# lucanest/Phyloformer

Hardware: AMD Instinct MI355X
Metric: alignments/sec, 60-leaf/500-site LG+GC-like MSAs, Phyloformer forward (pf.ckpt) (higher is better)
Workload: dtype f16x3-split MFMA (two fp16 limbs per operand, 3 passes), fp32 accumulate/residual

## Files before the change

### phyloformer_amd/csrc/pf_device.hip.h

```cpp
#pragma once
#include <hip/hip_runtime.h>
#include <stdint.h>

#include "pf_layout.h"

namespace pfk {

typedef float f32x4 __attribute__((ext_vector_type(4)));
typedef float f32x16 __attribute__((ext_vector_type(16)));
#if PF_F16
typedef _Float16 h16_t;
#define PF_MFMA(a, b, c) __builtin_amdgcn_mfma_f32_32x32x16_f16((a), (b), (c), 0, 0, 0)
#define PF_DOT2C "v_dot2c_f32_f16"
#define PF_CVT_PK "v_cvt_pk_f16_f32"
#define PF_NEG1_LO 0x0000bc00u
#define PF_NEG1_HI 0xbc000000u
#else
typedef __bf16 h16_t;
#define PF_MFMA(a, b, c) __builtin_amdgcn_mfma_f32_32x32x16_bf16((a), (b), (c), 0, 0, 0)
#define PF_DOT2C "v_dot2c_f32_bf16"
#define PF_CVT_PK "v_cvt_pk_bf16_f32"
#define PF_NEG1_LO 0x0000bf80u
#define PF_NEG1_HI 0xbf800000u
#endif
// ... 296 lines not shown
    int nt_aln;
    int slots_aln;
    size_t trash_tok;
    int store_x_last;
    unsigned long long* prof;
    int ablate;
    float* sitemap;
    const float* w;
};

enum { MODE_FIRST = 0, MODE_MID = 1, MODE_LAST = 2, MODE_MID0 = 3, MODE_LAST_FOLD = 4 };

struct TilePos { int b, kt, r0, l0; };
template <bool FLAT>
__device__ __forceinline__ TilePos tile_pos(const MainArgs& a, int task, int ntiles) {
    TilePos q;
    q.b = task / a.nt_aln;
    q.kt = task - q.b * a.nt_aln;
    if (FLAT) { const int tok0 = q.kt * 32; q.r0 = tok0 / a.Lloc; q.l0 = tok0 - q.r0 * a.Lloc; }
    else { q.r0 = q.kt / ntiles; q.l0 = (q.kt - q.r0 * ntiles) * 32; }
    return q;
}
template <bool FLAT>
__device__ __forceinline__ TilePos tile_next(const MainArgs& a, TilePos q) {
    if (++q.kt == a.nt_aln) { q.b++; q.kt = 0; q.r0 = 0; q.l0 = 0; return q; }
    q.l0 += 32;
    if (q.l0 >= a.Lloc) { q.l0 = FLAT ? q.l0 - a.Lloc : 0; q.r0++; }
    return q;
}
struct LanePos { size_t tok0; int toff, l, nvalid, wrap; bool valid, in_r1; };
template <bool FLAT>
__device__ __forceinline__ LanePos lane_pos(const MainArgs& a, const TilePos& q, int t) {
    LanePos o;
    o.tok0 = ((size_t)q.b * a.P + q.r0) * a.Lloc + q.l0;
    const int left = FLAT ? a.P * a.Lloc - q.kt * 32 : a.Lloc - q.l0;
    o.nvalid = min(32, left);
    o.wrap = (FLAT && q.r0 + 1 < a.P) ? min(32, a.Lloc - q.l0) : 32;
    o.valid = t < o.nvalid;
    o.toff = min(t, o.nvalid - 1);
    o.in_r1 = o.toff >= o.wrap;
    o.l = q.l0 + o.toff - (o.in_r1 ? a.Lloc : 0);
    return o;
}
__device__ __forceinline__ void part_range(int flat, int pr, int nparts, int P, int L, int slots_aln, long* first, int* count) {
    if (!flat) { *first = (long)pr * nparts; *count = nparts; return; }
    const int b = pr / P, p = pr - b * P;
    const int k0 = (int)(((long)p * L) >> 5), k1 = (int)((((long)p + 1) * L - 1) >> 5);
    *first = (long)b * slots_aln + k0 + p;
    *count = k1 - k0 + 1;
}

template <int LO, int HI>
__device__ __forceinline__ void image_to_lds(const frag_t* src, unsigned char* smem) {
    static_assert(LO % 64 == 0 && HI % 64 == 0, "the image is copied in whole waves");
    const int wv = threadIdx.x >> 6, ln = threadIdx.x & 63;
#pragma unroll
    for (int k = 0; k < (HI - LO + MAIN_THREADS - 1) / MAIN_THREADS; ++k) {
        const int f0 = LO + k * MAIN_THREADS + wv * 64;
        if (f0 < HI) __builtin_amdgcn_global_load_lds(src + f0 + ln, smem + (size_t)f0 * 16, 16, 0, 0);
    }
}

template <int MODE, bool FLAT, bool SITEMAP = false, bool WEIGHTED = false>
__global__ void __launch_bounds__(MAIN_THREADS, MAIN_WAVES / 4) k_main(MainArgs a) {
    constexpr bool LAST = MODE == MODE_LAST || MODE == MODE_LAST_FOLD;
    constexpr bool FOLD = MODE == MODE_LAST_FOLD;
    static_assert(!SITEMAP || LAST, "the site map is the head's: last block only");
    static_assert(!WEIGHTED || (!SITEMAP && MODE != MODE_FIRST), "weighted launches: blocks' own modes, no site map");
    extern __shared__ __attribute__((aligned(16))) unsigned char smem[];
    lds_frag_t lw = (lds_frag_t)smem;
    lds_f32_t lc = (lds_f32_t)(smem + FRAG_END * 16);

    {
        const float cv = a.consts[min((int)threadIdx.x, CONST_LEN - 1)];
        if (FOLD) {
            image_to_lds<FRAG_W1, FRAG_W2>(a.wimg, smem);
            image_to_lds<FRAG_WO, FRAG_U + U_FRAGS>(a.wimg, smem);
        } else {
            image_to_lds<(MODE == MODE_FIRST) ? FRAG_WV : 0, LAST ? FRAG_WV : FRAG_END>(a.wimg, smem);
        }
        static_assert(CONST_LEN <= MAIN_THREADS, "one constant per thread");
        if (threadIdx.x < CONST_LEN) reinterpret_cast<float*>(smem + FRAG_END * 16)[threadIdx.x] = cv;
        asm volatile("s_waitcnt vmcnt(0)" ::: "memory");
    }
    __syncthreads();

    const int lane = threadIdx.x & 63;
    const int wave = __builtin_amdgcn_readfirstlane(threadIdx.x >> 6);
    const int t = lane & 31;
    const int h = lane >> 5;
    const int ntiles = (a.Lloc + 31) >> 5;
    const int ntasks = a.B * a.nt_aln;
    if (wave >= MAIN_WAVES / 2) __builtin_amdgcn_s_setprio(1);
    unsigned long long tacc[6] = {0, 0, 0, 0, 0, 0}, tprev = 0;
#define PF_TICK(k) do { if (a.prof) { const unsigned long long tn_ = __builtin_amdgcn_s_memtime(); tacc[k] += tn_ - tprev; tprev = tn_; } } while (0)
    if (a.prof) tprev = __builtin_amdgcn_s_memtime();
    lds_frag_t w1p = lw + FRAG_W1 + lane;
    lds_frag_t w2p = lw + FRAG_W2 + lane;
    lds_frag_t wop = lw + FRAG_WO + lane;
    lds_frag_t qkp = lw + FRAG_QK + h * 8 + (t & 7);
    lds_f32_t lch = lc + 4 * h;
    PF_OPAQUE(wop); PF_OPAQUE(qkp); PF_OPAQUE(lch);
    lds_frag_t wvp = wop + (FRAG_WV - FRAG_WO);
    lds_f32_t luh = (lds_f32_t)(smem + FRAG_U * 16) + 16 * h;

    {
        const int nwaves = gridDim.x * MAIN_WAVES;
#ifndef PF_RUN_MAX
#define PF_RUN_MAX 8
#endif
        const int run = max(1, min(PF_RUN_MAX, ntasks / (nwaves * 8)));
        int run0 = (blockIdx.x * MAIN_WAVES + wave) * run;
        const int task0 = run0, task1 = ntasks;
        TilePos cur = tile_pos<FLAT>(a, min(task0, ntasks - 1), ntiles);
        int frag_row = -1;
        frag_t mfr[4];
        f32x4 rqv = {0.f, 0.f, 0.f, 0.f};
        f32x4 px[8], pctx[8], pqr, pqc;
        int pri = 0, prj = 0;
        auto prefetch = [&](const TilePos& np) {
            const LanePos nl = lane_pos<FLAT>(a, np, t);
            const int ll = nl.l, pb = np.b;
            const size_t tk = nl.tok0 + nl.toff;
            if (MODE == MODE_MID0) {
                const uint8_t* ib = a.idx + (size_t)pb * a.N * a.Lloc + ll;
                const int pp = np.r0 + (nl.in_r1 ? 1 : 0);
                pri = residue(ib[(size_t)a.pair_i[pp] * a.Lloc]);
                prj = residue(ib[(size_t)a.pair_j[pp] * a.Lloc]);
            } else {
                const f32x4* xp = reinterpret_cast<const f32x4*>(a.x + tk * 64 + 4 * h);
#pragma unroll
                for (int g = 0; g < 8; ++g) px[g] = xp[2 * g];
            }
            pqr = *reinterpret_cast<const f32x4*>(a.qrow + tk * 4);
            pqc = *reinterpret_cast<const f32x4*>(a.qcol + tk * 4);
            if (MODE != MODE_FIRST) {
                int hq = h;
                asm volatile("" : "+v"(hq));
                const f32x4* cp = reinterpret_cast<const f32x4*>(a.ctx + ((size_t)pb * a.Lloc + ll) * 64 + 4 * hq);
#pragma unroll
                for (int g = 0; g < 8; ++g) pctx[g] = cp[2 * g];
            }
        };
        if (MODE != MODE_FIRST && task0 < task1) prefetch(cur);

        for (int task = task0; task < task1;) {
            const int b = cur.b;
            const int row = b * a.P + cur.r0;
            int ntask = task + 1;
            TilePos nxt = tile_next<FLAT>(a, cur);
            if (ntask == run0 + run) {
                run0 += nwaves * run;
                ntask = run0;
                if (ntask < task1) nxt = tile_pos<FLAT>(a, ntask, ntiles);
            }
            const LanePos lp = lane_pos<FLAT>(a, cur, t);
            const bool straddle = lp.wrap < 32;
            int ai = 0, aj = 0;
            if (MODE == MODE_FIRST) { const int pp = cur.r0 + (lp.in_r1 ? 1 : 0); ai = a.pair_i[pp]; aj = a.pair_j[pp]; }
            auto load_mfr = [&](int r) {
                const frag_t* mf = a.mfrag + (size_t)r * 128 + t;
#pragma unroll
                for (int q = 0; q < 4; ++q) mfr[q] = mf[q * 32];
                typedef const f32x4 __attribute__((address_space(4)))* const_f32x4_t;
                rqv = *(const_f32x4_t)(unsigned long long)(a.rq + (size_t)__builtin_amdgcn_readfirstlane(r) * 4);
                frag_row = r;
            };
            if (MODE != MODE_FIRST && row != frag_row) load_mfr(row);
            const bool valid = lp.valid;
            const int lc_ = lp.l;
            const size_t tok = lp.tok0 + lp.toff;
            float x[32];
            float zh[4] = {0.f, 0.f, 0.f, 0.f};
            float wt = 1.f;
            if (WEIGHTED && LAST) wt = a.w[(size_t)b * a.Lloc + lc_];

            if (MODE == MODE_FIRST) {
                const int ri = residue(a.idx[((size_t)b * a.N + ai) * a.Lloc + lc_]);
                const int rj = residue(a.idx[((size_t)b * a.N + aj) * a.Lloc + lc_]);
                const f32x4* ti = reinterpret_cast<const f32x4*>(a.table + ri * 64 + 4 * h);
                const f32x4* tj = reinterpret_cast<const f32x4*>(a.table + rj * 64 + 4 * h);
#pragma unroll
                for (int g = 0; g < 8; ++g) {
                    f32x4 u = ti[2 * g], w = tj[2 * g];
#pragma unroll
                    for (int i = 0; i < 4; ++i) x[4 * g + i] = u[i] + w[i];
                }
            } else {
                if (MODE == MODE_MID0) {
                    const f32x4* ti = reinterpret_cast<const f32x4*>(a.table + pri * 64 + 4 * h);
                    const f32x4* tj = reinterpret_cast<const f32x4*>(a.table + prj * 64 + 4 * h);
#pragma unroll
                    for (int g = 0; g < 8; ++g) {
                        const f32x4 u = ti[2 * g], w = tj[2 * g];
#pragma unroll
                        for (int i = 0; i < 4; ++i) x[4 * g + i] = u[i] + w[i];
                    }
                } else {
#pragma unroll
                    for (int g = 0; g < 8; ++g)
#pragma unroll
                        for (int i = 0; i < 4; ++i) x[4 * g + i] = px[g][i];
                }
                PF_TICK(0);
                if (!(a.ablate & 8)) {
                    f32x16 ya[2];
#pragma unroll
                    for (int j = 0; j < 32; ++j) ya[j >> 4][j & 15] = x[j];
                    {
                        const f32x4 qr = pqr;
                        auto mix = [&](const bool mine) {
                            float v[8];
#pragma unroll
                            for (int i = 0; i < 4; ++i) v[i] = mine ? qr[i] * rqv[i] : 0.f;
                            v[4] = v[5] = mine ? 1.f : 0.f;
                            v[6] = v[7] = 0.f;
                            frag_t qb_hi, qb_lo;
                            split8(v, qb_hi, qb_lo);
#pragma unroll
                            for (int To = 0; To < 2; ++To) mfma3(ya[To], mfr[To * 2], mfr[To * 2 + 1], qb_hi, qb_lo, To == 1);
                        };
                        mix(h == 0 && !lp.in_r1);
                        if (straddle) {
                            load_mfr(row + 1);
                            mix(h == 0 && lp.in_r1);
                        }
                    }
                    {
                        const f32x4 qc = pqc * COLAPPLY_B_SCALE;
                        float o[32];
#pragma unroll
                        for (int g = 0; g < 8; ++g) {
                            const f32x4 u = pctx[g];
#pragma unroll
                            for (int i = 0; i < 4; ++i) o[4 * g + i] = u[i] * qc[g >> 1];
                        }
#pragma unroll
                        for (int s = 0; s < 4; ++s) {
                            frag_t ob_hi, ob_lo;
                            split8(&o[8 * s], ob_hi, ob_lo);
#pragma unroll
                            for (int To = 0; To < 2; ++To) {
                                lds_frag_t f = wop + ((To * 4 + s) * 2) * 64;
                                const frag_t a_hi = f[0], a_lo = f[64];
                                mfma3(ya[To], a_hi, a_lo, ob_hi, ob_lo, To == 1);
                            }
                        }
                    }
#pragma unroll
                    for (int j = 0; j < 32; ++j) x[j] = ya[j >> 4][j & 15];
                }

                PF_TICK(1);
                if (FOLD) {
#pragma unroll
                    for (int g = 0; g < 8; ++g) {
                        const f32x4 w4 = *(lds_f32x4_t)(lch + CONST_HW + 8 * g);
#pragma unroll
                        for (int i = 0; i < 4; ++i) zh[i] = fmaf(w4[i], x[4 * g + i], zh[i]);
                    }
                }
                if (FOLD && !(a.ablate & 16)) {
                    frag_t xb_hi[4], xb_lo[4];
                    {
                        float xn[32];
                        ln_pair(x, xn);
#pragma unroll
                        for (int s = 0; s < 4; ++s) split8(&xn[8 * s], xb_hi[s], xb_lo[s]);
                    }
                    if (ntask < task1) prefetch(nxt);
                    PF_TICK(2);
#pragma unroll 1
                    for (int T = 0; T < 8; ++T) {
                        f32x16 ha;
                        lds_frag_t f1 = w1p + T * 512;
                        lds_f32_t bp = lch + CONST_B1 + 32 * T;
                        lds_f32_t up = luh + 32 * T;
                        PF_OPAQUE(f1); PF_OPAQUE(bp); PF_OPAQUE(up);
// ... 43 lines not shown
                            frag_t nh, nl;
                            if (s < 3) { nh = f1[(s + 1) * 128]; nl = f1[(s + 1) * 128 + 64]; }
                            else { nh = f2[0]; nl = f2[64]; }
                            mfma3(ha, fh, fl, xb_hi[s], xb_lo[s]);
                            fh = nh; fl = nl;
                        }
                        frag_t g_hi[2], g_lo[2];
                        gelu_split8(ha, 0, g_hi[0], g_lo[0]);
                        gelu_split8(ha, 8, g_hi[1], g_lo[1]);
#pragma unroll
                        for (int st = 0; st < 4; ++st) {
                            const int u = st >> 1, To = st & 1;
                            frag_t nh = fh, nl = fl;
                            if (st < 3) {
                                const int nu = (st + 1) >> 1, nTo = (st + 1) & 1;
                                nh = f2[(nTo * 32 + nu * 2) * 64];
                                nl = f2[(nTo * 32 + nu * 2) * 64 + 64];
                            }
                            mfma3(oa[To], fh, fl, g_hi[u], g_lo[u], To == 1);
                            fh = nh; fl = nl;
                        }
                    }
                    PF_TICK(3);
#pragma unroll
                    for (int j = 0; j < 32; ++j) x[j] = oa[j >> 4][j & 15];
                }
            }

            if (!LAST && !(a.ablate & 4)) {
                frag_t wl[8];
#pragma unroll
                for (int i = WVLO_LDS; i < 8; ++i) wl[i] = a.wv_lo[i * 64 + lane];
                if (WEIGHTED) wt = a.w[(size_t)b * a.Lloc + lc_];
                __builtin_amdgcn_sched_barrier(0);
                {
                    const size_t stok = valid ? tok : a.trash_tok + t;
                    f32x4* xo = reinterpret_cast<f32x4*>(a.x + stok * 64 + 4 * h);
#pragma unroll
                    for (int g = 0; g < 8; ++g) {
                        f32x4 u = {x[4 * g], x[4 * g + 1], x[4 * g + 2], x[4 * g + 3]};
                        xo[2 * g] = u;
                    }
                }
                if (a.ablate & 32) { cur = nxt; task = ntask; continue; }
                f32x16 va[3];
                {
                    float xn[32];
                    ln_pair(x, xn);
                    frag_t xb_hi[4], xb_lo[4];
#pragma unroll
                    for (int s = 0; s < 4; ++s) split8(&xn[8 * s], xb_hi[s], xb_lo[s]);
#pragma unroll
                    for (int s = 0; s < 4; ++s) {
                        const frag_t q_hi = qkp[(s * 2) * 16], q_lo = qkp[(s * 2 + 1) * 16];
                        if (s == 0) mfma3_zero(va[2], q_hi, q_lo, xb_hi[s], xb_lo[s]);
                        else mfma3(va[2], q_hi, q_lo, xb_hi[s], xb_lo[s]);
                    }
#pragma unroll
                    for (int s = 0; s < 4; ++s)
#pragma unroll
                        for (int T = 0; T < 2; ++T) {
                            const frag_t f_hi = wvp[(T * 4 + s) * 64];
                            const frag_t f_lo = T * 4 + s < WVLO_LDS ? wvp[(FRAG_WVLO - FRAG_WV) + (T * 4 + s) * 64] : wl[T * 4 + s];
                            if (s == 0) mfma3_zero(va[T], f_hi, f_lo, xb_hi[s], xb_lo[s], T == 1);
                            else mfma3(va[T], f_hi, f_lo, xb_hi[s], xb_lo[s], T == 1);
                        }
                }
#pragma unroll
                for (int r = 0; r < 4; ++r) va[2][r] += lc[CONST_BQK + 4 * h + r];
                float qk[4], ot[4];
#pragma unroll
                for (int i = 0; i < 4; ++i) qk[i] = elu1_fast(va[2][i]);
#pragma unroll
                for (int i = 0; i < 4; ++i) ot[i] = pair_other(qk[i], h);
                float qn[4], kn[4];
#pragma unroll
                for (int i = 0; i < 4; ++i) {
                    qn[i] = h ? ot[i] : qk[i];
                    kn[i] = h ? qk[i] : ot[i];
                }
                {
                    const size_t stok = valid ? tok : a.trash_tok + t;
                    f32x4 qs = {qn[0], qn[1], qn[2], qn[3]};
                    *reinterpret_cast<f32x4*>(a.qrow + stok * 4) = qs;
                }
                const long slot0 = (long)b * a.slots_aln + cur.kt + (FLAT ? cur.r0 : 0);
                for (int part = 0; part < (straddle ? 2 : 1); ++part) {
                    float* sp = a.spart + (size_t)(slot0 + part) * SROW;
                    const float vm = (valid && lp.in_r1 == (part == 1)) ? (WEIGHTED ? wt : 1.f) : 0.f;
                    float km[4];
#pragma unroll
                    for (int i = 0; i < 4; ++i) km[i] = kn[i] * vm;
                    {
                        float qk8[8];
#pragma unroll
                        for (int i = 0; i < 4; ++i) { qk8[i] = vm * qn[i]; qk8[4 + i] = km[i]; }
                        const float sqk = treduce8(qk8, t);
                        if (lane < 8) sp[64 + lane] = sqk;
                    }
                    {
                        float kv[32];
#pragma unroll
                        for (int j = 0; j < 32; ++j) kv[j] = km[j >> 3] * va[j >> 4][j & 15];
                        sp[kmap(t, h)] = treduce32(kv, t);
                    }
                }
            } else if (LAST) {
                float z = 0.f;
                if (FOLD) {
                    z = pair_sum((zh[0] + zh[1]) + (zh[2] + zh[3])) + lc[CONST_C0];
                } else {
#pragma unroll
                    for (int g = 0; g < 8; ++g) {
                        const f32x4 w4 = *(lds_f32x4_t)(lch + CONST_HW + 8 * g);
#pragma unroll
                        for (int i = 0; i < 4; ++i) z = fmaf(w4[i], x[4 * g + i], z);
                    }
                    z = pair_sum(z) + lc[CONST_HB];
                }
                const float spz = softplus20(z);
                const long slot0 = (long)b * a.slots_aln + cur.kt + (FLAT ? cur.r0 : 0);
                for (int part = 0; part < (straddle ? 2 : 1); ++part) {
// ... 614 lines not shown
                    n[u] = gg < a.G ? (min(a.npairs, (gg + 1) * per) - gg * per + a.sub - 1) / a.sub : 0;
                    nmax = max(nmax, n[u]);
                    pg[u] = pp + (size_t)gg * a.S * gs;
                    t[u] = 0.f;
                }
                for (int s = 0; s < nmax; s += 4) {
                    float v[GU][4];
#pragma unroll
                    for (int u = 0; u < GU; ++u)
#pragma unroll
                        for (int q = 0; q < 4; ++q)
                            v[u][q] = s + q < n[u] ? pg[u][(size_t)(s + q) * gs] : 0.f;
#pragma unroll
                    for (int u = 0; u < GU; ++u) t[u] = (((t[u] + v[u][0]) + v[u][1]) + v[u][2]) + v[u][3];
                }
#pragma unroll
                for (int u = 0; u < GU; ++u)
                    if (g + u < a.G) acc += t[u];
            }
        } else {
            const float* pp = a.part + ((size_t)b * a.G * a.Lloc + l) * CPART + i;
            int g = 0;
            for (; g + 4 <= a.G; g += 4) {
                const float v0 = pp[(size_t)g * gs], v1 = pp[(size_t)(g + 1) * gs], v2 = pp[(size_t)(g + 2) * gs],
                            v3 = pp[(size_t)(g + 3) * gs];
                acc = (((acc + v0) + v1) + v2) + v3;
            }
            for (; g < a.G; ++g) acc += pp[(size_t)g * gs];
        }
        zs[i] = acc;
    }
    __syncthreads();
    if (i < 256) {
        const float* z = zs + (hd >> 4) * 64 + 16 * quarter;
        float acc = 0.f;
#pragma unroll
        for (int k = 0; k < 16; ++k) acc = fmaf(w[k], z[k], acc);
        dp[quarter][hd] = acc;
    }
    __syncthreads();
    if (i < 64) {
        const int hh = hd >> 4;
        const float acc = ((dp[0][hd] + dp[1][hd]) + dp[2][hd]) + dp[3][hd];
        const float sq = zs[256 + hh], sk = zs[260 + hh];
        a.ctx[(size_t)site * 64 + hd] = (acc + a.bv[hd] * sk) / sk * (a.P / sq);
    }
}

__global__ void k_accumulate(float* dst, const float* src, size_t n) {
    const size_t i = (size_t)blockIdx.x * blockDim.x + threadIdx.x;
    if (i < n) dst[i] += src[i];
}

__global__ void k_selftest(float* out) {
    const int lane = threadIdx.x;
    out[lane] = pair_sum((float)lane);
    out[64 + lane] = pair_other((float)lane, lane >> 5);
    out[128 + lane] = row16_sum((float)lane);
    out[192 + lane] = half32_sum((float)lane);
    frag_t A1, A2, Bf;
    const int m = lane & 31, kg = lane >> 5;
#pragma unroll
    for (int i = 0; i < 8; ++i) {
        const int k = 8 * kg + i;
        A1[i] = (h16_t)(float)(m + 32 * (k % 8));
        A2[i] = (h16_t)(float)k;
        Bf[i] = (h16_t)((k == (m & 15)) ? 1.f : 0.f);
    }
    f32x16 acc1, acc2;
#pragma unroll
    for (int r = 0; r < 16; ++r) { acc1[r] = 0.f; acc2[r] = 0.f; }
    acc1 = PF_MFMA(A1, Bf, acc1);
    acc2 = PF_MFMA(A2, Bf, acc2);
#pragma unroll
    for (int r = 0; r < 16; ++r) {
        out[256 + lane * 16 + r] = acc1[r];
        out[1280 + lane * 16 + r] = acc2[r];
    }
}

#endif

}
```

### phyloformer_amd/csrc/pf_host_prep.h

```cpp
#pragma once
#include <algorithm>
#include <cmath>
#include <cstdint>
#include <cstring>
#include <vector>

#include "pf_layout.h"

namespace pfhost {
using namespace pfk;

inline uint16_t f2bf(float f) {
    uint32_t u;
    std::memcpy(&u, &f, 4);
    if ((u & 0x7fffffffu) > 0x7f800000u) return uint16_t((u >> 16) | 0x40);
    u += 0x7fffu + ((u >> 16) & 1u);
    return uint16_t(u >> 16);
}
inline float bf2f(uint16_t b) {
    uint32_t u = uint32_t(b) << 16;
    float f;
    std::memcpy(&f, &u, 4);
    return f;
}
// ... 5 lines not shown
    if (u >= 0x7f800000u) return uint16_t(sign | 0x7c00u | (u > 0x7f800000u ? 0x200u : 0u));
    if (u >= 0x477ff000u) return uint16_t(sign | 0x7c00u);
    if (u < 0x33000001u) return sign;
    const int e = int(u >> 23) - 127;
    uint32_t m = (u & 0x7fffffu) | 0x800000u;
    int shift = (e < -14) ? (13 + (-14 - e)) : 13;
    const uint32_t half = 1u << (shift - 1), rest = m & ((1u << shift) - 1);
    uint32_t r = m >> shift;
    if (rest > half || (rest == half && (r & 1u))) ++r;
    const uint32_t out = (e < -14) ? r : (uint32_t(e + 14) << 10) + r;
    return uint16_t(sign | out);
}
inline float h2f(uint16_t hbits) {
    const uint32_t sign = uint32_t(hbits & 0x8000u) << 16;
    const int e = (hbits >> 10) & 0x1f;
    const uint32_t m = hbits & 0x3ffu;
    float mag;
    if (e == 0) mag = std::ldexp((float)m, -24);
    else if (e == 31) mag = m ? NAN : INFINITY;
    else mag = std::ldexp((float)(m | 0x400u), e - 25);
    uint32_t u;
    std::memcpy(&u, &mag, 4);
    u |= sign;
    std::memcpy(&mag, &u, 4);
    return mag;
}
#if PF_F16
inline uint16_t f2x(float f) { return f2h(f); }
inline float x2f(uint16_t b) { return h2f(b); }
#else
inline uint16_t f2x(float f) { return f2bf(f); }
inline float x2f(uint16_t b) { return bf2f(b); }
#endif
inline int kmap_h(int j, int h) { return 8 * (j >> 2) + 4 * h + (j & 3); }

inline void pack_frags(const float* W, int M, int K, int Mpad, uint16_t* out, float scale = 1.f) {
    const int nT = Mpad / 32, nS = K / 16;
    for (int T = 0; T < nT; ++T)
        for (int s = 0; s < nS; ++s)
            for (int lane = 0; lane < 64; ++lane)
                for (int i = 0; i < 8; ++i) {
                    const int m = 32 * T + (lane & 31), k = kmap_h(8 * s + i, lane >> 5);
                    const float w = (m < M) ? W[(size_t)m * K + k] * scale : 0.f;
                    const uint16_t hi = f2x(w);
                    const uint16_t lo = f2x(w - x2f(hi));
                    const size_t base = ((size_t)(T * nS + s) * 2) * 64;
                    out[(base + lane) * 8 + i] = hi;
                    out[(base + 64 + lane) * 8 + i] = lo;
                }
}

inline void pack_qk_frags(const float* wq, const float* wk, uint16_t* qk) {
    for (int s = 0; s < 4; ++s)
        for (int kg = 0; kg < 2; ++kg)
            for (int m = 0; m < 8; ++m)
                for (int i = 0; i < 8; ++i) {
                    const int k = kmap_h(8 * s + i, kg);
                    const float w = (m < 4) ? wq[(size_t)m * E + k] : wk[(size_t)(m - 4) * E + k];
                    const uint16_t hi = f2x(w), lo = f2x(w - x2f(hi));
                    qk[(((size_t)s * 2 + 0) * 16 + kg * 8 + m) * 8 + i] = hi;
                    qk[(((size_t)s * 2 + 1) * 16 + kg * 8 + m) * 8 + i] = lo;
                }
}

inline void pack_row_stats(const float* wv, const float* wq, const float* wk, uint16_t* img_tail ,
                    uint16_t* wv_lo) {
    std::vector<uint16_t> full((size_t)2 * 4 * 2 * 64 * 8);
    pack_frags(wv, E, E, E, full.data());
    for (int T = 0; T < 2; ++T)
        for (int s = 0; s < 4; ++s)
            for (int lane = 0; lane < 64; ++lane)
                for (int i = 0; i < 8; ++i) {
                    const size_t src = (((size_t)(T * 4 + s) * 2) * 64 + lane) * 8 + i;
                    const size_t dst = ((size_t)(T * 4 + s) * 64 + lane) * 8 + i;
                    img_tail[dst] = full[src];
                    wv_lo[dst] = full[src + 64 * 8];
                }
    pack_qk_frags(wq, wk, img_tail + (size_t)(FRAG_QK - FRAG_WV) * 8);
}

inline void fold_head(const float* w2 , const float* b2, const float* hw, float hb, double w2_scale,
                      float* u_img , float* c0) {
    for (int T = 0; T < FF / 32; ++T)
        for (int h = 0; h < 2; ++h)
            for (int r = 0; r < 16; ++r) {
                const int k = 32 * T + kmap_h(r, h);
                double acc = 0.0;
                for (int c = 0; c < E; ++c) acc += (double)hw[c] * (double)w2[(size_t)c * FF + k];
                u_img[(T * 2 + h) * 16 + r] = (float)(acc * w2_scale);
            }
    double acc = (double)hb;
    for (int c = 0; c < E; ++c) acc += (double)hw[c] * (double)b2[c];
    *c0 = (float)acc;
}

struct AttnHost {
    const float *g, *b, *wq, *bq, *wk, *bk, *wv, *bv, *wo, *bo;
};
struct FfnHost {
    const float *g, *b, *w1, *b1, *w2, *b2;
};

struct BlobView {
    const float *emb_w, *emb_b;
    std::vector<AttnHost> row, col;
    std::vector<FfnHost> ffn;
    const float *head_w, *head_b;
    size_t len;
};
inline BlobView read_blob(const float* blob, int n_blocks, int E, int NH) {
    BlobView v{};
    const size_t e = (size_t)E, h = (size_t)NH;
    auto take = [&](size_t n) { const float* p = blob ? blob + v.len : nullptr; v.len += n; return p; };
    auto attn = [&] {
        AttnHost a;
// ... 112 lines not shown
```

### phyloformer_amd/csrc/pf_layout.h

```cpp
#pragma once

#ifndef PF_F16
#define PF_F16 1
#endif

namespace pfk {

constexpr int E = 64;
constexpr int NH = 4;
constexpr int HD = 16;
constexpr int FF = 256;
constexpr int NA = 22;
constexpr int SROW = 72;
constexpr int MROW = 4 * 64;
constexpr float LN_EPS = 1e-5f;

constexpr int FRAG_W1 = 0;
constexpr int FRAG_W2 = FRAG_W1 + 8 * 4 * 2 * 64;
constexpr int FRAG_WO = FRAG_W2 + 2 * 16 * 2 * 64;
constexpr int FRAG_WV = FRAG_WO + 2 * 4 * 2 * 64;
constexpr int FRAG_QK = FRAG_WV + 2 * 4 * 64;
#ifndef PF_WVLO_LDS
#define PF_WVLO_LDS 4
#endif
constexpr int WVLO_LDS = PF_WVLO_LDS;
constexpr int FRAG_WVLO = FRAG_QK + 4 * 2 * 16;
constexpr int FRAG_END = FRAG_WVLO + WVLO_LDS * 64;
constexpr int FRAG_U = FRAG_WV;
constexpr int U_FRAGS = FF * 4 / 16;
static_assert(FRAG_U + U_FRAGS <= FRAG_END, "the folded head fits the last block's tail");
constexpr int WVLO_FRAGS = 2 * 4 * 64;
constexpr int CONST_B1 = 0, CONST_B2 = 256, CONST_BQK = 320, CONST_HW = 328, CONST_HB = 392,
              CONST_C0 = 393, CONST_BOC = 400;
constexpr int CONST_LEN = 464;
constexpr int MAIN_LDS_BYTES = FRAG_END * 16 + CONST_LEN * 4;
constexpr int MFRAG_PER_PAIR = 2 * 2 * 32;

constexpr int MAIN_THREADS = 512;
constexpr int MAIN_WAVES = MAIN_THREADS / 64;

constexpr int PAIRTAB_ROWS = 22 * 22, PAIRTAB_W = 72;

}
```

### phyloformer_amd/csrc/pf_lib.hip

```cpp
#include <hip/hip_runtime.h>
#include <dlfcn.h>

#include <algorithm>
#include <cmath>
#include <cstdarg>
#include <cstdio>
#include <cstdlib>
#include <cstring>
#include <functional>
#include <map>
#include <mutex>
#include <string>
#include <type_traits>
#include <vector>

#include "../../include/phyloformer_amd.h"
#include "pf_device.hip.h"
#include "pf_mha.hip.h"
#include "pf_precise.hip.h"
#include "pf_generic.hip.h"
#include "pf_boot.hip.h"
#include "pf_sites.hip.h"
#include "pf_sitemap.hip.h"
#include "pf_sites_host.h"
// ... 603 lines not shown
        EmbedArgs e{r.d_idx, h->pair_i, h->pair_j, h->pair_table, h->table, x0, r.w.qrow, r.w.srow,
                    r.B, r.N, r.P, r.Lloc, h->bad_idx_dev, r.d_w};
        const int ntasks = r.B * r.P, wpb = EMBED_THREADS / 64;
        const int grid = std::max(1, std::min(h->prop.multiProcessorCount, (ntasks + wpb - 1) / wpb));
        ProfScope ps(h, K_EMBED);
        if (r.d_w) hipLaunchKernelGGL(k_embed<true>, dim3(grid), dim3(EMBED_THREADS), EMBED_LDS_BYTES, h->cur, e);
        else hipLaunchKernelGGL(k_embed<false>, dim3(grid), dim3(EMBED_THREADS), EMBED_LDS_BYTES, h->cur, e);
        HIPCHK(h, hipGetLastError());
    }
    if (h->debug_keep) return save_tap(h, "x0", r.w.x, (size_t)r.B * r.P * r.Lloc * 64);
    return PF_OK;
}

int tiles_of(int Lloc) { return (Lloc + 31) / 32; }

int launch_rowsum(pf_handle* h, const ShardRun& r, RowStats* rs) {
    if (rs->p == r.w.srow) return PF_OK;
    const int n = r.B * r.P * SROW;
    if (!r.Lloc) { *rs = RowStats{r.w.srow, 1, 0}; return zero_fill(h, r.w.srow, n); }
    ProfScope ps(h, K_ROWFIN);
    hipLaunchKernelGGL(k_rowsum, dim3((n + 255) / 256), dim3(256), 0, h->cur, rs->p, r.w.srow, r.B * r.P, rs->nparts,
                       rs->flat, r.P, r.Lloc, r.tp.slots_aln);
    HIPCHK(h, hipGetLastError());
    *rs = RowStats{r.w.srow, 1, 0};
    return PF_OK;
}

int launch_outsum(pf_handle* h, const ShardRun& r) {
    const int n = r.B * r.P;
    if (!r.Lloc) return zero_fill(h, r.d_out, n);
    ProfScope ps(h, K_ROWFIN);
    const TilePlan& tp = r.tp;
    hipLaunchKernelGGL(k_outsum, dim3((n + 255) / 256), dim3(256), 0, h->cur, r.w.outpart, r.d_out, n,
                       tiles_of(r.Lloc), 1.0f / (float)r.L_total, tp.flat, r.P, r.Lloc, tp.slots_aln, r.d_wst);
    HIPCHK(h, hipGetLastError());
    return PF_OK;
}

RowStats main_stats(const ShardRun& r) { return RowStats{r.w.spart, tiles_of(r.Lloc), r.tp.flat}; }

RowStats first_stats(pf_handle* h, const ShardRun& r) {
    return h->embed_mfma ? main_stats(r) : RowStats{r.w.srow, 1, 0};
}

int phase_block(pf_handle* h, const ShardRun& r, int k, RowStats rs) {
    if (!r.Lloc) return PF_OK;
    const BlockDev& d = h->blk[k];
    const Workspace& w = r.w;
    const int B = r.B, P = r.P, Lloc = r.Lloc;
    int rc;
    if (h->debug_keep) {
        if ((rc = launch_rowsum(h, r, &rs))) return rc;
        if ((rc = save_tap(h, "srow" + std::to_string(k), rs.p, (size_t)B * P * SROW))) return rc;
    }
    {
        RowFinArgs a{rs.p, w.mrow, reinterpret_cast<frag_t*>(w.mfrag),
                     d.row_woT, d.row_bv, d.row_bo, d.col_bo,
                     B * P, rs.nparts, (float)r.L_total, rs.flat, P, Lloc, r.tp.slots_aln, 1};
        const int groups = (B * P + 3) / 4;
        a.iters = std::max(1, std::min(16, groups / (4 * 8 * std::max(1, h->prop.multiProcessorCount))));
        a.rq = w.rq;
        a.b_scale = 1.f;
        for (long lim = 16384; lim < (long)r.L_total && a.b_scale > 1.f / 256.f; lim *= 2) a.b_scale *= 0.5f;
        a.a_scale = 1.f / a.b_scale;
        a.wst = r.d_wst;
        ProfScope ps(h, K_ROWFIN);
        hipLaunchKernelGGL(k_rowfin, dim3((groups + a.iters - 1) / a.iters), dim3(256), 0, h->cur, a);
        HIPCHK(h, hipGetLastError());
    }
    {
        ColStatsArgs a{w.x, w.qrow, w.mrow, w.qcol, w.part, d.col_wqk, d.col_bqk, d.row_bo, B, P, Lloc, w.G, (Lloc + 31) / 32,
                       w.sub, w.S, w.fine, h->table, r.d_idx, h->pair_i, h->pair_j, r.N};
        ProfScope ps(h, K_COLSTATS);
        const unsigned nblk = (unsigned)(B * a.nchunks * w.nparts());
        if (k == 0 && x0_on_the_fly(h))
            hipLaunchKernelGGL((k_colstats<true, 0, 16>), dim3(nblk), dim3(256), 0, h->cur, a);
        else if (h->colstats_ring)
            hipLaunchKernelGGL((k_colstats<false, PF_CS_RING, PF_CS_MT>), dim3(nblk), dim3(256), 0, h->cur, a);
        else
            hipLaunchKernelGGL((k_colstats<false, 0, 16>), dim3(nblk), dim3(256), 0, h->cur, a);
        HIPCHK(h, hipGetLastError());
    }
    {
        ColFinArgs a{w.part, w.ctx, d.col_wvT, d.col_bv, B, Lloc, w.G, (float)P, P, w.sub, w.S, w.fine};
        ProfScope ps(h, K_COLFIN);
        hipLaunchKernelGGL(k_colfin, dim3(B * Lloc), dim3(COLFIN_THREADS), 0, h->cur, a);
        HIPCHK(h, hipGetLastError());
    }
    if (h->debug_keep) {
        if ((rc = save_tap(h, "ctx" + std::to_string(k), w.ctx, (size_t)B * Lloc * 64))) return rc;
        if ((rc = save_tap(h, "mrow" + std::to_string(k), w.mrow, (size_t)B * P * MROW))) return rc;
    }
    MainArgs m = main_args(h, r);
    m.wimg = reinterpret_cast<const frag_t*>(d.wimg);
    m.consts = d.consts;
    if (k + 1 < h->n_blocks) {
        m.wv_lo = reinterpret_cast<const frag_t*>(h->blk[k + 1].wv_lo);
        const bool first = k == 0 && x0_on_the_fly(h);
        if (r.d_w) rc = first ? launch_main<MODE_MID0, false, true>(h, m, K_MAIN) : launch_main<MODE_MID, false, true>(h, m, K_MAIN);
        else rc = first ? launch_main<MODE_MID0>(h, m, K_MAIN) : launch_main<MODE_MID>(h, m, K_MAIN);
        if (rc) return rc;
    } else {
        m.wv_lo = nullptr;
        if (h->phase_prof_last) m.prof = h->phase_prof;
        m.sitemap = r.d_smap;
        if (!h->head_fold) {
// ... 2183 lines not shown
    if (!h) return PF_EINVAL;
    if (domain) *domain = h->prop.pciDomainID;
    if (bus) *bus = h->prop.pciBusID;
    if (device) *device = h->prop.pciDeviceID;
    return PF_OK;
}

int pf_forward_shards_emulated(pf_handle_t* h, const uint8_t* idx, int32_t B, int32_t N, int32_t L,
                               int32_t nshards, float* out) {
    if (!h) return PF_EINVAL;
    int rc = check_dims(h, B, N, L, L);
    if (rc) return rc;
    if (nshards < 1 || nshards > 64 || !idx || !out) return fail(h, PF_EINVAL, "bad shard count or null buffer");
    HIPCHK(h, hipSetDevice(h->device));
    if (const F64Path* f = f64_path_of(h, N, L)) return forward_shards_emulated_f64(h, *f, idx, B, N, L, nshards, out);
    if ((rc = ensure_pairs(h, N))) return rc;
    const int P = N * (N - 1) / 2;
    ShardStage stage(h);
    if ((rc = stage.upload(idx, B, N, L, nshards))) return rc;
    std::vector<ShardRun> runs;
    for (const ShardStage::Shard& s : stage.shards) {
        ShardRun r{{}, s.d_idx, nullptr, B, N, P, s.Lloc, L, tile_plan(h, P, s.Lloc), h->stream, {}};
        size_t off[WS_BUFS];
        char* ws = (char*)stage.alloc(workspace_bytes(h, B, P, r.Lloc, &r.w, off));
        r.d_out = (float*)stage.alloc((size_t)B * P * sizeof(float));
        if (!ws || !r.d_out) return fail(h, PF_ENOMEM, "shard workspace allocation failed");
        carve_workspace(ws, off, &r.w);
        runs.push_back(r);
    }
    float* total = (float*)stage.alloc((size_t)B * P * SROW * sizeof(float));
    if (!total) return fail(h, PF_ENOMEM, "shard sum buffer");
    auto reduce = [&](bool site_sums) -> int {
        const size_t count = (size_t)B * P * (site_sums ? 1 : SROW);
        for (ShardRun& r : runs)
            if (!site_sums && (rc = launch_rowsum(h, r, &r.rs))) return rc;
        hipMemsetAsync(total, 0, count * sizeof(float), h->stream);
        for (ShardRun& r : runs) {
            hipLaunchKernelGGL(k_accumulate, dim3((unsigned)((count + 255) / 256)), dim3(256), 0, h->stream,
                               total, site_sums ? r.d_out : r.w.srow, count);
            r.rs = RowStats{total, 1, 0};
        }
        return PF_OK;
    };
    rc = schedule(h, runs.data(), runs.size(), reduce);
    if (!rc && (hipMemcpyAsync(out, total, (size_t)B * P * sizeof(float), hipMemcpyDeviceToHost, h->stream) != hipSuccess ||
                hipStreamSynchronize(h->stream) != hipSuccess))
        rc = fail(h, PF_EHIP, "result copy failed");
    return rc;
}

int pf_selftest(pf_handle_t* h, float* out) {
    if (!h || !out) return PF_EINVAL;
    float* d = nullptr;
    HIPCHK(h, hipMalloc((void**)&d, 2304 * sizeof(float)));
    hipLaunchKernelGGL(k_selftest, dim3(1), dim3(64), 0, h->stream, d);
    HIPCHK(h, hipGetLastError());
    HIPCHK(h, hipMemcpyAsync(out, d, 2304 * sizeof(float), hipMemcpyDeviceToHost, h->stream));
    HIPCHK(h, hipStreamSynchronize(h->stream));
    hipFree(d);
    return PF_OK;
}

struct pf_mha {
    pf_handle* h = nullptr;
    float* wfrag = nullptr;
    float* bias = nullptr;
    std::vector<DeviceBuffer*> buffers;
    Buffer<char> ws{buffers};
    Buffer<float> d_x{buffers}, d_y{buffers};
};

int pf_mha_create(pf_handle_t* h, const pf_mha_weights_t* w, pf_mha_t** out) {
    if (!h || !w || !out) return PF_EINVAL;
    if (w->n_heads != MHA_H || w->embed_dim != E)
        return fail(h, PF_EINVAL, "softmax attention kernels are specialised for embed_dim 64 / 4 heads, got %d / %d",
                    w->embed_dim, w->n_heads);
    const float* ws[4] = {w->wq, w->wk, w->wv, w->wo};
    const float* bs[4] = {w->bq, w->bk, w->bv, w->bo};
    std::vector<uint16_t> img((size_t)MHA_WTOTAL * 8);
    std::vector<float> bias(4 * E);
    for (int i = 0; i < 4; ++i) {
        if (!ws[i] || !bs[i]) return fail(h, PF_EINVAL, "pf_mha_create: NULL weight pointer");
        std::copy(bs[i], bs[i] + E, bias.begin() + i * E);
    }
    pack_frags(w->wq, E, E, E, img.data());
    pack_frags(w->wk, E, E, E, img.data() + (size_t)MHA_OFF_WK * 8);
    pack_frags(w->wv, E, E, E, img.data() + (size_t)MHA_OFF_WV * 8);
    pack_frags(w->wo, E, E, E, img.data() + (size_t)MHA_OFF_WO * 8);
    HIPCHK(h, hipSetDevice(h->device));
    pf_mha* m = new pf_mha();
    m->h = h;
    void* p = nullptr;
    if (hipMalloc(&p, img.size() * 2) != hipSuccess) { delete m; return fail(h, PF_ENOMEM, "pf_mha_create: hipMalloc failed"); }
    m->wfrag = (float*)p;
    if (hipMalloc(&p, bias.size() * 4) != hipSuccess) { hipFree(m->wfrag); delete m; return fail(h, PF_ENOMEM, "pf_mha_create: hipMalloc failed"); }
    m->bias = (float*)p;
    if (hipMemcpy(m->wfrag, img.data(), img.size() * 2, hipMemcpyHostToDevice) != hipSuccess ||
        hipMemcpy(m->bias, bias.data(), bias.size() * 4, hipMemcpyHostToDevice) != hipSuccess) {
        hipFree(m->wfrag); hipFree(m->bias); delete m;
        return fail(h, PF_EHIP, "pf_mha_create: weight upload failed");
    }
    *out = m;
    return PF_OK;
}

int pf_mha_destroy(pf_mha_t* m) {
    if (!m) return PF_OK;
    hipSetDevice(m->h->device);
    hipStreamSynchronize(m->h->stream);
    hipFree(m->wfrag); hipFree(m->bias);
// ... 64 lines not shown
```

### phyloformer_amd/engine.py

```python
from __future__ import annotations

import ctypes as C
import os
from typing import Dict, Optional, Tuple

import numpy as np

from .weights import ModelWeights

HERE = os.path.dirname(os.path.abspath(__file__))
LIB_PATH = os.path.join(HERE, "libphyloformer_amd.so")
ABI_VERSION = 5
UNIQUE_ID_BYTES = 256

PF_OK, PF_EINVAL, PF_EHIP, PF_ERCCL, PF_ENOMEM, PF_ESTATE = 0, -1, -2, -3, -4, -5


def _refuse_single_sequence(B: int, N: int):
    if N == 1 and B >= 1:
        raise RuntimeError(f"cannot reshape tensor of 0 elements into shape [{B}, -1, 0, 64] because the unspecified "
                           "dimension size -1 can be any value and is ambiguous")


class EngineError(RuntimeError):
# ... 651 lines not shown
                               L_total: int, d_out: int):
        self._check(self._lib.pf_forward_sharded_device(
            self._h, C.c_void_p(d_idx), B, N, l_begin, l_end, L_total, C.c_void_p(d_out)))

    def synchronize(self):
        self._check(self._lib.pf_synchronize(self._h))

    def unique_id(self) -> bytes:
        buf = C.create_string_buffer(UNIQUE_ID_BYTES)
        rc = self._lib.pf_comm_unique_id(buf)
        if rc != PF_OK:
            raise EngineError(rc, (self._lib.pf_last_error(None) or b"").decode())
        return buf.raw

    def comm_init(self, unique_id: Optional[bytes], rank: int, world: int):
        buf = C.create_string_buffer(unique_id, UNIQUE_ID_BYTES) if unique_id else None
        self._check(self._lib.pf_comm_init(self._h, buf, rank, world))
        self.rank, self.world = rank, world

    def comm_destroy(self):
        self._check(self._lib.pf_comm_destroy(self._h))
        self.rank, self.world = 0, 1

    def collective_count(self) -> int:
        return self.profile_get("collectives")[0]

    def rechecked_count(self) -> int:
        return self.profile_get("rechecked")[0]

    def comm_info(self) -> dict:
        buf = C.create_string_buffer(512)
        ver = C.c_int32()
        rc = self._lib.pf_comm_info(buf, 512, C.byref(ver))
        if rc != PF_OK:
            raise EngineError(rc, (self._lib.pf_last_error(None) or b"").decode())
        return {"library": buf.value.decode(), "version": int(ver.value)}

    def profile_reset(self):
        self._check(self._lib.pf_profile_reset(self._h))

    def profile_get(self, kernel: str) -> Tuple[int, float]:
        n = C.c_int64()
        ms = C.c_double()
        self._check(self._lib.pf_profile_get(self._h, kernel.encode(), C.byref(n), C.byref(ms)))
        return n.value, ms.value

    def debug_read(self, name: str) -> np.ndarray:
        n = self._check(self._lib.pf_debug_read(self._h, name.encode(), None, 0))
        out = np.empty(n, dtype=np.float32)
        self._check(self._lib.pf_debug_read(self._h, name.encode(), out.ctypes.data, n))
        return out

    def selftest(self) -> np.ndarray:
        out = np.empty(2304, dtype=np.float32)
        self._check(self._lib.pf_selftest(self._h, out.ctypes.data))
        return out
```

Measured before the change: 543.6.

## Pack hi/lo weight limbs into one MFMA operand to cut split-precision passes

The QK projection now packs the weight hi and lo limbs into the row halves of a single fragment. Two MFMAs (against the activation's lo and hi limbs) then produce hi*x and lo*x in separate output rows, which are summed afterwards, replacing three or four MFMAs per step. The pair-mix path likewise uses a lane-wide mfrag layout of two fragments per row, zeroing qb_lo on the upper half to drop the lo*lo term, and issues four MFMAs with fewer per-lane loads. Because the QK image is no longer a multiple of 64 fragments, a scalar tail copy into LDS is added. Selftest cases for the new packing tricks are also added. The risks are the changed accumulation order and dependence on the host packing matching the device indexing.

Measured after the change: 548.9, median of 6. About the same (+1.0%).

```diff
diff --git a/phyloformer_amd/csrc/pf_device.hip.h b/phyloformer_amd/csrc/pf_device.hip.h
--- a/phyloformer_amd/csrc/pf_device.hip.h
+++ b/phyloformer_amd/csrc/pf_device.hip.h
@@ -372,13 +372,15 @@
 
 template <int LO, int HI>
 __device__ __forceinline__ void image_to_lds(const frag_t* src, unsigned char* smem) {
-    static_assert(LO % 64 == 0 && HI % 64 == 0, "the image is copied in whole waves");
+    static_assert(LO % 64 == 0, "the image is copied in whole waves");
+    constexpr int HIW = HI - (HI - LO) % 64;
     const int wv = threadIdx.x >> 6, ln = threadIdx.x & 63;
 #pragma unroll
-    for (int k = 0; k < (HI - LO + MAIN_THREADS - 1) / MAIN_THREADS; ++k) {
+    for (int k = 0; k < (HIW - LO + MAIN_THREADS - 1) / MAIN_THREADS; ++k) {
         const int f0 = LO + k * MAIN_THREADS + wv * 64;
-        if (f0 < HI) __builtin_amdgcn_global_load_lds(src + f0 + ln, smem + (size_t)f0 * 16, 16, 0, 0);
-    }
+        if (f0 < HIW) __builtin_amdgcn_global_load_lds(src + f0 + ln, smem + (size_t)f0 * 16, 16, 0, 0);
+    }
+    if (HIW < HI && (int)threadIdx.x < HI - HIW) reinterpret_cast<frag_t*>(smem)[HIW + threadIdx.x] = src[HIW + threadIdx.x];
 }
 
 template <int MODE, bool FLAT, bool SITEMAP = false, bool WEIGHTED = false>
@@ -418,7 +420,7 @@
     lds_frag_t w1p = lw + FRAG_W1 + lane;
     lds_frag_t w2p = lw + FRAG_W2 + lane;
     lds_frag_t wop = lw + FRAG_WO + lane;
-    lds_frag_t qkp = lw + FRAG_QK + h * 8 + (t & 7);
+    lds_frag_t qkp = lw + FRAG_QK + (t < 16 ? h * 16 + t : 32 + h);
     lds_f32_t lch = lc + 4 * h;
     PF_OPAQUE(wop); PF_OPAQUE(qkp); PF_OPAQUE(lch);
     lds_frag_t wvp = wop + (FRAG_WV - FRAG_WO);
@@ -434,7 +436,7 @@
         const int task0 = run0, task1 = ntasks;
         TilePos cur = tile_pos<FLAT>(a, min(task0, ntasks - 1), ntiles);
         int frag_row = -1;
-        frag_t mfr[4];
+        frag_t mfr[2];
         f32x4 rqv = {0.f, 0.f, 0.f, 0.f};
         f32x4 px[8], pctx[8], pqr, pqc;
         int pri = 0, prj = 0;
@@ -479,9 +481,9 @@
             int ai = 0, aj = 0;
             if (MODE == MODE_FIRST) { const int pp = cur.r0 + (lp.in_r1 ? 1 : 0); ai = a.pair_i[pp]; aj = a.pair_j[pp]; }
             auto load_mfr = [&](int r) {
-                const frag_t* mf = a.mfrag + (size_t)r * 128 + t;
-#pragma unroll
-                for (int q = 0; q < 4; ++q) mfr[q] = mf[q * 32];
+                const frag_t* mf = a.mfrag + (size_t)r * MFRAG_PER_PAIR + lane;
+#pragma unroll
+                for (int To = 0; To < 2; ++To) mfr[To] = mf[To * 64];
                 typedef const f32x4 __attribute__((address_space(4)))* const_f32x4_t;
                 rqv = *(const_f32x4_t)(unsigned long long)(a.rq + (size_t)__builtin_amdgcn_readfirstlane(r) * 4);
                 frag_row = r;
@@ -537,13 +539,16 @@
                             v[6] = v[7] = 0.f;
                             frag_t qb_hi, qb_lo;
                             split8(v, qb_hi, qb_lo);
-#pragma unroll
-                            for (int To = 0; To < 2; ++To) mfma3(ya[To], mfr[To * 2], mfr[To * 2 + 1], qb_hi, qb_lo, To == 1);
+                            if (h) qb_lo = zero_frag();
+                            ya[0] = PF_MFMA(mfr[0], qb_lo, ya[0]);
+                            ya[0] = PF_MFMA(mfr[0], qb_hi, ya[0]);
+                            ya[1] = PF_MFMA(mfr[1], qb_hi, ya[1]);
+                            ya[1] = PF_MFMA(mfr[1], qb_lo, ya[1]);
                         };
-                        mix(h == 0 && !lp.in_r1);
+                        mix(!lp.in_r1);
                         if (straddle) {
                             load_mfr(row + 1);
-                            mix(h == 0 && lp.in_r1);
+                            mix(lp.in_r1);
                         }
                     }
                     {
@@ -693,9 +698,14 @@
                     for (int s = 0; s < 4; ++s) split8(&xn[8 * s], xb_hi[s], xb_lo[s]);
 #pragma unroll
                     for (int s = 0; s < 4; ++s) {
-                        const frag_t q_hi = qkp[(s * 2) * 16], q_lo = qkp[(s * 2 + 1) * 16];
-                        if (s == 0) mfma3_zero(va[2], q_hi, q_lo, xb_hi[s], xb_lo[s]);
-                        else mfma3(va[2], q_hi, q_lo, xb_hi[s], xb_lo[s]);
+                        const frag_t q_hl = qkp[s * QK_STEP];
+                        if (s == 0) {
+                            const f32x16 z = {0.f, 0.f, 0.f, 0.f, 0.f, 0.f, 0.f, 0.f, 0.f, 0.f, 0.f, 0.f, 0.f, 0.f, 0.f, 0.f};
+                            va[2] = PF_MFMA(q_hl, xb_lo[s], z);
+                        } else {
+                            va[2] = PF_MFMA(q_hl, xb_lo[s], va[2]);
+                        }
+                        va[2] = PF_MFMA(q_hl, xb_hi[s], va[2]);
                     }
 #pragma unroll
                     for (int s = 0; s < 4; ++s)
@@ -708,7 +718,7 @@
                         }
                 }
 #pragma unroll
-                for (int r = 0; r < 4; ++r) va[2][r] += lc[CONST_BQK + 4 * h + r];
+                for (int r = 0; r < 4; ++r) va[2][r] = (va[2][r] + va[2][r + 4]) + lc[CONST_BQK + 4 * h + r];
                 float qk[4], ot[4];
 #pragma unroll
                 for (int i = 0; i < 4; ++i) qk[i] = elu1_fast(va[2][i]);
@@ -1429,6 +1439,7 @@
     if (i < n) dst[i] += src[i];
 }
 
+constexpr int SELFTEST_LEN = 5376;
 __global__ void k_selftest(float* out) {
     const int lane = threadIdx.x;
     out[lane] = pair_sum((float)lane);
@@ -1454,6 +1465,27 @@
         out[256 + lane * 16 + r] = acc1[r];
         out[1280 + lane * 16 + r] = acc2[r];
     }
+    frag_t A3, A5, Bbb, Bb0;
+#pragma unroll
+    for (int i = 0; i < 8; ++i) {
+        A3[i] = (h16_t)(kg ? (float)(i + 1) * 0.0625f : (float)(m + 32 * i));
+        const float a5 = (float)(16 * (m & 7) + 8 * kg + i);
+        A5[i] = (h16_t)(m < 8 ? a5 : m < 16 ? a5 * (1.f / 512.f) : 0.f);
+        Bbb[i] = (h16_t)((i == (m & 7)) ? 1.f : 0.f);
+        Bb0[i] = (h16_t)((kg == 0 && i == (m & 7)) ? 1.f : 0.f);
+    }
+    f32x16 acc3, acc4, acc5;
+#pragma unroll
+    for (int r = 0; r < 16; ++r) { acc3[r] = 0.f; acc4[r] = 0.f; acc5[r] = 0.f; }
+    acc3 = PF_MFMA(A3, Bbb, acc3);
+    acc4 = PF_MFMA(A3, Bb0, acc4);
+    acc5 = PF_MFMA(A5, Bf, acc5);
+#pragma unroll
+    for (int r = 0; r < 16; ++r) {
+        out[2304 + lane * 16 + r] = acc3[r];
+        out[3328 + lane * 16 + r] = acc4[r];
+        out[4352 + lane * 16 + r] = acc5[r];
+    }
 }
 
 #endif
diff --git a/phyloformer_amd/csrc/pf_host_prep.h b/phyloformer_amd/csrc/pf_host_prep.h
--- a/phyloformer_amd/csrc/pf_host_prep.h
+++ b/phyloformer_amd/csrc/pf_host_prep.h
@@ -81,15 +81,17 @@
 
 inline void pack_qk_frags(const float* wq, const float* wk, uint16_t* qk) {
     for (int s = 0; s < 4; ++s)
-        for (int kg = 0; kg < 2; ++kg)
+        for (int kg = 0; kg < 2; ++kg) {
             for (int m = 0; m < 8; ++m)
                 for (int i = 0; i < 8; ++i) {
                     const int k = kmap_h(8 * s + i, kg);
                     const float w = (m < 4) ? wq[(size_t)m * E + k] : wk[(size_t)(m - 4) * E + k];
                     const uint16_t hi = f2x(w), lo = f2x(w - x2f(hi));
-                    qk[(((size_t)s * 2 + 0) * 16 + kg * 8 + m) * 8 + i] = hi;
-                    qk[(((size_t)s * 2 + 1) * 16 + kg * 8 + m) * 8 + i] = lo;
-                }
+                    qk[((size_t)s * QK_STEP + kg * 16 + m) * 8 + i] = hi;
+                    qk[((size_t)s * QK_STEP + kg * 16 + 8 + m) * 8 + i] = lo;
+                }
+            for (int i = 0; i < 8; ++i) qk[((size_t)s * QK_STEP + 32 + kg) * 8 + i] = 0;
+        }
 }
 
 inline void pack_row_stats(const float* wv, const float* wq, const float* wk, uint16_t* img_tail ,
diff --git a/phyloformer_amd/csrc/pf_layout.h b/phyloformer_amd/csrc/pf_layout.h
--- a/phyloformer_amd/csrc/pf_layout.h
+++ b/phyloformer_amd/csrc/pf_layout.h
@@ -20,11 +20,12 @@
 constexpr int FRAG_WO = FRAG_W2 + 2 * 16 * 2 * 64;
 constexpr int FRAG_WV = FRAG_WO + 2 * 4 * 2 * 64;
 constexpr int FRAG_QK = FRAG_WV + 2 * 4 * 64;
+constexpr int QK_STEP = 2 * 16 + 2;
 #ifndef PF_WVLO_LDS
 #define PF_WVLO_LDS 4
 #endif
 constexpr int WVLO_LDS = PF_WVLO_LDS;
-constexpr int FRAG_WVLO = FRAG_QK + 4 * 2 * 16;
+constexpr int FRAG_WVLO = FRAG_QK + 4 * QK_STEP;
 constexpr int FRAG_END = FRAG_WVLO + WVLO_LDS * 64;
 constexpr int FRAG_U = FRAG_WV;
 constexpr int U_FRAGS = FF * 4 / 16;
@@ -34,7 +35,8 @@
               CONST_C0 = 393, CONST_BOC = 400;
 constexpr int CONST_LEN = 464;
 constexpr int MAIN_LDS_BYTES = FRAG_END * 16 + CONST_LEN * 4;
-constexpr int MFRAG_PER_PAIR = 2 * 2 * 32;
+static_assert(MAIN_LDS_BYTES <= 160 * 1024, "k_main's LDS image and constants fit one CU's LDS");
+constexpr int MFRAG_PER_PAIR = 2 * 64;
 
 constexpr int MAIN_THREADS = 512;
 constexpr int MAIN_WAVES = MAIN_THREADS / 64;
diff --git a/phyloformer_amd/csrc/pf_lib.hip b/phyloformer_amd/csrc/pf_lib.hip
--- a/phyloformer_amd/csrc/pf_lib.hip
+++ b/phyloformer_amd/csrc/pf_lib.hip
@@ -679,6 +679,7 @@
     if (h->debug_keep) {
         if ((rc = launch_rowsum(h, r, &rs))) return rc;
         if ((rc = save_tap(h, "srow" + std::to_string(k), rs.p, (size_t)B * P * SROW))) return rc;
+        if ((rc = save_tap(h, "qrow" + std::to_string(k), w.qrow, (size_t)B * P * Lloc * 4))) return rc;
     }
     {
         RowFinArgs a{rs.p, w.mrow, reinterpret_cast<frag_t*>(w.mfrag),
@@ -2968,10 +2969,10 @@
 int pf_selftest(pf_handle_t* h, float* out) {
     if (!h || !out) return PF_EINVAL;
     float* d = nullptr;
-    HIPCHK(h, hipMalloc((void**)&d, 2304 * sizeof(float)));
+    HIPCHK(h, hipMalloc((void**)&d, SELFTEST_LEN * sizeof(float)));
     hipLaunchKernelGGL(k_selftest, dim3(1), dim3(64), 0, h->stream, d);
     HIPCHK(h, hipGetLastError());
-    HIPCHK(h, hipMemcpyAsync(out, d, 2304 * sizeof(float), hipMemcpyDeviceToHost, h->stream));
+    HIPCHK(h, hipMemcpyAsync(out, d, SELFTEST_LEN * sizeof(float), hipMemcpyDeviceToHost, h->stream));
     HIPCHK(h, hipStreamSynchronize(h->stream));
     hipFree(d);
     return PF_OK;
diff --git a/phyloformer_amd/engine.py b/phyloformer_amd/engine.py
--- a/phyloformer_amd/engine.py
+++ b/phyloformer_amd/engine.py
@@ -727,6 +727,6 @@
         return out
 
     def selftest(self) -> np.ndarray:
-        out = np.empty(2304, dtype=np.float32)
+        out = np.empty(5376, dtype=np.float32)
         self._check(self._lib.pf_selftest(self._h, out.ctypes.data))
         return out
```
